# olegroshka/vae-channel-dynamics

Measured on AMD Instinct MI355X. Metric: images/sec SDXL-VAE train step @256x256 (tracking on), higher is better.
Workload: dtype f32

## Files before the change

vae-channel-dynamics_amd/csrc/wgrad3_upwino.hip:

```cpp
#include "wino_common.h"
#include <algorithm>
#include <type_traits>

#ifndef VAE_UPWGRAD_X3
#define VAE_UPWGRAD_X3 1
#endif
#if VAE_UPWGRAD_X3
#include "bf16_frag.h"
#endif
#ifndef VAE_UPWGRAD_PRIO
#define VAE_UPWGRAD_PRIO 1
#endif

namespace {

constexpr int GCI = 32, GCO = 128, NPOS = 9, GNT = 512, GNB = GCO / 32;
constexpr int XSX = 12;
constexpr int XSY = 20;
constexpr int SXF = 3 * GCI * XSX;
constexpr int SYF = 2 * GCO * XSY;
constexpr int GSTAGE = SXF + SYF;
#if VAE_UPWGRAD_X3
constexpr int GPAIR = 2 * GSTAGE;
constexpr int GLDS = 2 * GPAIR * (int)sizeof(float);
extern __shared__ __attribute__((aligned(16))) float upwgrad_lds[];
#endif

__global__ __launch_bounds__(GNT, 2) void wgrad3_upwino_kernel(vae_wgrad_args p, int strips, int64_t nunits) {
#if VAE_UPWGRAD_X3
  float* const smem = upwgrad_lds;
#else
  __shared__ __attribute__((aligned(16))) float smem[2 * GSTAGE];
#endif

  const int tid = threadIdx.x, lane = tid & 63, wave = tid >> 6;
  const int lr = lane & 31, lh = lane >> 5;
  const vae_conv_geom g = p.g;
  const int tilesN = p.N / GCI, ntile = tilesN * (p.M / GCO);
  const wino::SplitTile wg = wino::split_tile_of_workgroup<false>(blockIdx.x, p.nsplit, ntile);
  const int tile = wg.tile, split = wg.split;
  const int tm = tile / tilesN, tn = tile % tilesN;
  const int m0 = tm * GCO, n0 = tn * GCI;
  const wino::UnitRange ur = wino::unit_range(nunits, p.nsplit, split);
  const int64_t ubeg = ur.ubeg;
  const int nu = ur.nu;
  const int upi = g.Hs * strips;
  const bool do_bias = (p.bias_partial != nullptr) && tn == 0;

  const int xx = tid & 15, yq = tid >> 4;
  const bool xrole = tid < 240;
  const int xq = tid & 7, xc = (tid >> 3) % 10, xr = tid / 80;
  const auto rsX = VAE_BUF_RSRC(p.X, (size_t)g.B * g.Hs * g.Ws * g.Cs * 4u);
  const auto rsY = VAE_BUF_RSRC(p.dY, (size_t)g.B * g.Ho * g.Wo * p.ldy * 4u);
  struct Stg {
    f32x4 rx, ry[2];
  };
  const f32x4 z4 = {0.f, 0.f, 0.f, 0.f};
  Stg s0{z4, {z4, z4}}, s1{z4, {z4, z4}};
  f32x4 bsum = z4;
  int ub = (int)(ubeg / upi), urow = (int)((ubeg - (int64_t)ub * upi) / strips), ustrip = (int)((ubeg - (int64_t)ub * upi) % strips);
  const unsigned rowY = (unsigned)g.Wo * p.ldy * 4u;
  auto load_unit = [&](int k, Stg& r) {
    const bool ok = k < nu;
    const int b = ub, i = urow, x0 = ustrip * 8;
    if (++ustrip == strips) {
      ustrip = 0;
      if (++urow == g.Hs) {
        urow = 0;
        ++ub;
      }
    }
    const int hy = i - 1 + xr, hx = x0 - 1 + xc;
    const bool xin = ok && xrole && ((unsigned)hy < (unsigned)g.Hs) && ((unsigned)hx < (unsigned)g.Ws);
    r.rx = VAE_BUF_LOAD4(rsX, xin ? (unsigned)(((b * g.Hs + hy) * g.Ws + hx) * g.Cs + n0 + 4 * xq) * 4u : BUF_OOB);
    const unsigned baseY = (unsigned)((b * g.Ho + 2 * i) * g.Wo + 2 * x0 + xx) * (unsigned)p.ldy * 4u + (unsigned)(m0 + 4 * yq) * 4u;
#pragma unroll
    for (int a = 0; a < 2; ++a) r.ry[a] = VAE_BUF_LOAD4(rsY, ok ? baseY + a * rowY : BUF_OOB);
  };
  auto store_unit = [&](float* st, const Stg& r) {
    float* sx = st;
    float* sy = st + SXF;
    if (xrole) {
#pragma unroll
      for (int e = 0; e < 4; ++e) sx[(xr * GCI + 4 * xq + e) * XSX + xc] = r.rx[e];
    }
#pragma unroll
    for (int a = 0; a < 2; ++a) {
#pragma unroll
      for (int e = 0; e < 4; ++e) sy[(a * GCO + 4 * yq + e) * XSY + xx] = r.ry[a][e];
      if (do_bias) bsum += r.ry[a];
    }
  };

  f32x16 acc[GNB], accx;
#pragma unroll
  for (int nb = 0; nb < GNB; ++nb)
#pragma unroll
    for (int e = 0; e < 16; ++e) acc[nb][e] = 0.f;
#pragma unroll
  for (int e = 0; e < 16; ++e) accx[e] = 0.f;

#if VAE_UPWGRAD_X3
  auto stage_pair = [&](float* st, int kp) __attribute__((always_inline)) {
    store_unit(st, s0);
    store_unit(st + GSTAGE, s1);
    load_unit(2 * kp + 2, s0);
    load_unit(2 * kp + 3, s1);
  };
  load_unit(0, s0);
  load_unit(1, s1);
  stage_pair(smem, 0);
  __syncthreads();
#else
  load_unit(0, s0);
  store_unit(smem, s0);
  load_unit(1, s1);
  __syncthreads();
#endif

  auto build_a = [&](auto PR, auto PC, const float* cx, f32x4& a4) {
    constexpr int pr = decltype(PR)::value, pc = decltype(PC)::value;
    constexpr int vr1 = pr == 0 ? 0 : 1, vr2 = pr == 0 ? 1 : 2;
    const int voff1 = (vr1 * GCI + lr) * XSX + 4 * lh, voff2 = (vr2 * GCI + lr) * XSX + 4 * lh;
    float rc[8];
#pragma unroll
    for (int c = 0; c < 2; ++c) {
      const f32x4 u1 = *reinterpret_cast<const f32x4*>(&cx[voff1 + 4 * c]);
      if (pr == 1) {
#pragma unroll
        for (int e = 0; e < 4; ++e) rc[4 * c + e] = u1[e];
      } else {
        const f32x4 u2 = *reinterpret_cast<const f32x4*>(&cx[voff2 + 4 * c]);
#pragma unroll
        for (int e = 0; e < 4; ++e) rc[4 * c + e] = u1[e] - u2[e];
      }
    }
#pragma unroll
    for (int e = 0; e < 4; ++e) a4[e] = pc == 0 ? rc[e] - rc[e + 1] : (pc == 1 ? rc[e + 1] : rc[e + 1] - rc[e + 2]);
  };
  auto build_b = [&](auto PR, auto PC, const float* cy, int nb, f32x4& b4) {
    constexpr int pr = decltype(PR)::value, pc = decltype(PC)::value;
    constexpr int dr1 = pr == 2 ? 1 : 0;
    const int doff = (dr1 * GCO + nb * 32 + lr) * XSY + 8 * lh;
    float rc[8];
#pragma unroll
    for (int c = 0; c < 2; ++c) {
      const f32x4 d0 = *reinterpret_cast<const f32x4*>(&cy[doff + 4 * c]);
      if (pr == 1) {
        const f32x4 d1 = *reinterpret_cast<const f32x4*>(&cy[doff + GCO * XSY + 4 * c]);
#pragma unroll
        for (int e = 0; e < 4; ++e) rc[4 * c + e] = d0[e] + d1[e];
      } else {
#pragma unroll
        for (int e = 0; e < 4; ++e) rc[4 * c + e] = d0[e];
      }
    }
#pragma unroll
    for (int e = 0; e < 4; ++e) b4[e] = pc == 0 ? rc[2 * e] : (pc == 1 ? rc[2 * e] + rc[2 * e + 1] : rc[2 * e + 1]);
  };
  using I2 = std::integral_constant<int, 2>;

  auto run = [&](auto PR, auto PC, auto EXTRA) {
    constexpr bool extra = decltype(EXTRA)::value;
#if VAE_UPWGRAD_X3
    auto step = [&](int kp) {
      const float* cst = smem + (kp & 1) * GPAIR;
      float* nst = smem + ((kp + 1) & 1) * GPAIR;
      Bf3 a3, bb;
      {
        f32x4 a0, a1;
        build_a(PR, PC, cst, a0);
        build_a(PR, PC, cst + GSTAGE, a1);
        a3 = split8(a0, a1);
      }
      if (extra) stage_pair(nst, kp + 1);
      __builtin_amdgcn_sched_barrier(0);
#pragma unroll
      for (int nb = 0; nb < GNB; ++nb) {
        if (nb == GNB - 1 && !extra) {
          __builtin_amdgcn_sched_barrier(0);
          stage_pair(nst, kp + 1);
          __builtin_amdgcn_sched_barrier(0);
        }
        f32x4 b0, b1;
        build_b(PR, PC, cst + SXF, nb, b0);
        build_b(PR, PC, cst + GSTAGE + SXF, nb, b1);
        bb = split8(b0, b1);
#pragma unroll
        for (int t = 0; t < 6; ++t) acc[nb] = mma_x3_term(t, a3.p, bb.p, acc[nb]);
      }
      if (extra) {
        f32x4 a0, a1, b0, b1;
        build_a(I2{}, I2{}, cst, a0);
        build_a(I2{}, I2{}, cst + GSTAGE, a1);
        build_b(I2{}, I2{}, cst + SXF, wave, b0);
        build_b(I2{}, I2{}, cst + GSTAGE + SXF, wave, b1);
        a3 = split8(a0, a1);
        bb = split8(b0, b1);
#pragma unroll
        for (int t = 0; t < 6; ++t) accx = mma_x3_term(t, a3.p, bb.p, accx);
      }
      __syncthreads();
    };
    const int np = (nu + 1) / 2;
    for (int kp = 0; kp < np; ++kp) step(kp);
#else
    auto step = [&](int k, const Stg& cur, Stg& nxt) {
      const float* cx = smem + (k & 1) * GSTAGE;
      const float* cy = cx + SXF;
      float* nst = smem + ((k + 1) & 1) * GSTAGE;
      f32x4 a4, bb[2];
      build_a(PR, PC, cx, a4);
      build_b(PR, PC, cy, 0, bb[0]);
#pragma unroll
      for (int nb = 0; nb < GNB; ++nb) {
        __builtin_amdgcn_sched_barrier(0);
        if (nb == 1) {
          load_unit(k + 2, nxt);
          __builtin_amdgcn_sched_barrier(0);
        }
        if (nb + 1 < GNB) build_b(PR, PC, cy, nb + 1, bb[(nb + 1) & 1]);
#pragma unroll
        for (int e = 0; e < 4; ++e) acc[nb] = __builtin_amdgcn_mfma_f32_32x32x2f32(a4[e], bb[nb & 1][e], acc[nb], 0, 0, 0);
        __builtin_amdgcn_sched_barrier(0);
      }
      if (extra) {
        f32x4 ax, bx;
        build_a(I2{}, I2{}, cx, ax);
        build_b(I2{}, I2{}, cy, wave, bx);
#pragma unroll
        for (int e = 0; e < 4; ++e) accx = __builtin_amdgcn_mfma_f32_32x32x2f32(ax[e], bx[e], accx, 0, 0, 0);
      }
      store_unit(nst, cur);
      __syncthreads();
    };
    int k = 0;
    for (; k + 1 < nu; k += 2) {
      step(k, s1, s0);
      step(k + 1, s0, s1);
    }
    if (k < nu) step(k, s1, s0);
#endif
  };
#if VAE_UPWGRAD_X3 && VAE_UPWGRAD_PRIO
  if (__builtin_amdgcn_readfirstlane(tid) >= 256) __builtin_amdgcn_s_setprio(1);
#endif
  {
    using I0 = std::integral_constant<int, 0>;
    using I1 = std::integral_constant<int, 1>;
    using T = std::true_type;
    using F_ = std::false_type;
    switch (wave) {
      case 0: run(I0{}, I0{}, T{}); break;
      case 1: run(I0{}, I1{}, T{}); break;
      case 2: run(I0{}, I2{}, T{}); break;
      case 3: run(I1{}, I0{}, T{}); break;
      case 4: run(I1{}, I1{}, F_{}); break;
      case 5: run(I1{}, I2{}, F_{}); break;
      case 6: run(I2{}, I0{}, F_{}); break;
      default: run(I2{}, I1{}, F_{}); break;
    }
  }
#if VAE_UPWGRAD_X3 && VAE_UPWGRAD_PRIO
  __builtin_amdgcn_s_setprio(0);
#endif

  float* __restrict__ O = p.partial + (int64_t)split * NPOS * p.N * p.M;
  wino::slab_store<GNB>(O, wave, p.N, p.M, n0, m0, 0, acc, lr, lh);
  if (wave < 4) wino::slab_store<1>(O, 8, p.N, p.M, n0, m0, wave, &accx, lr, lh);
  if (do_bias) wino::bias_tail(bsum, xx, p.bias_partial, (int64_t)split * p.M + m0 + 4 * yq);
}

}

bool wgrad3_upwino_eligible(const vae_wgrad_args& a) {
  const vae_conv_geom& g = a.g;
  if (!wino::wgrad_eligible_common(a, GCI, GCO) || a.x_bf16 || a.y_bf16 || a.xf != VAE_XF_NONE) return false;
  if (g.mode != VAE_MODE_UP2X || g.Ho != 2 * g.Hs || g.Wo != 2 * g.Ws) return false;
  return g.Ws % 8 == 0 && g.Cs >= a.N;
}

int64_t wgrad3_upwino_units(const vae_conv_geom& g) { return (int64_t)g.B * g.Hs * (g.Ws / 8); }

int launch_wgrad3_upwino(const vae_wgrad_args& a, hipStream_t st) {
  const vae_conv_geom& g = a.g;
  const int64_t nunits = wgrad3_upwino_units(g);
  dim3 grid((unsigned)((a.M / GCO) * (a.N / GCI) * a.nsplit), 1, 1);
#if VAE_UPWGRAD_X3
  VAE_RESERVE_LDS(wgrad3_upwino_kernel, GLDS, "wgrad3_upwino");
  hipLaunchKernelGGL(wgrad3_upwino_kernel, grid, dim3(GNT), GLDS, st, a, g.Ws / 8, nunits);
#else
  hipLaunchKernelGGL(wgrad3_upwino_kernel, grid, dim3(GNT), 0, st, a, g.Ws / 8, nunits);
#endif
  return 0;
}
```

Baseline: 120.0.

## Software-pipeline B-operand builds under MFMA in upsample Winograd wgrad kernel

Adds a pipelined step for the x3 bf16 path of the upsample Winograd weight-gradient kernel. The B operand for the next column block is built from LDS while the current block's MFMAs run, using a double-buffered register operand. Explicit sched_group_barrier patterns interleave MFMA, LDS reads and VALU work, and s_setprio raises wave priority around the MFMA section. This targets LDS-read and split latency sitting between matrix ops, at the cost of more live registers and a compiler-schedule-sensitive instruction mix.

```diff
diff --git a/vae-channel-dynamics_amd/csrc/wgrad3_upwino.hip b/vae-channel-dynamics_amd/csrc/wgrad3_upwino.hip
--- a/vae-channel-dynamics_amd/csrc/wgrad3_upwino.hip
+++ b/vae-channel-dynamics_amd/csrc/wgrad3_upwino.hip
@@ -10,6 +10,12 @@
 #endif
 #ifndef VAE_UPWGRAD_PRIO
 #define VAE_UPWGRAD_PRIO 1
+#endif
+#ifndef VAE_UPWGRAD_PIPE_PRIO
+#define VAE_UPWGRAD_PIPE_PRIO 1
+#endif
+#ifndef VAE_UPWGRAD_PIPE
+#define VAE_UPWGRAD_PIPE 1
 #endif
 
 namespace {
@@ -163,6 +169,71 @@
   auto run = [&](auto PR, auto PC, auto EXTRA) {
     constexpr bool extra = decltype(EXTRA)::value;
 #if VAE_UPWGRAD_X3
+#if VAE_UPWGRAD_PIPE
+    auto step = [&](int kp) {
+      const float* cst = smem + (kp & 1) * GPAIR;
+      float* nst = smem + ((kp + 1) & 1) * GPAIR;
+      Bf3 a3, ax3, bb[2];
+      auto operand = [&](auto PR_, auto PC_, int nb, Bf3& o) {
+        f32x4 b0, b1;
+        build_b(PR_, PC_, cst + SXF, nb, b0);
+        build_b(PR_, PC_, cst + GSTAGE + SXF, nb, b1);
+        o = split8(b0, b1);
+      };
+      {
+        f32x4 a0, a1;
+        build_a(PR, PC, cst, a0);
+        build_a(PR, PC, cst + GSTAGE, a1);
+        a3 = split8(a0, a1);
+      }
+      if (extra) stage_pair(nst, kp + 1);
+      operand(PR, PC, 0, bb[0]);
+      __builtin_amdgcn_sched_barrier(0);
+      if (VAE_UPWGRAD_PIPE_PRIO && extra) __builtin_amdgcn_s_setprio(2);
+      constexpr int pr = decltype(PR)::value, pc = decltype(PC)::value;
+      constexpr int nrd = pr == 1 ? 4 : 2;
+      constexpr int gv = (44 + (pr == 1 ? 16 : 0) + (pc == 1 ? 8 : 0) + 5) / 6;
+#pragma unroll
+      for (int nb = 0; nb < GNB; ++nb) {
+        if (nb == GNB - 1 && !extra) {
+          stage_pair(nst, kp + 1);
+          __builtin_amdgcn_sched_barrier(0);
+        }
+        if (nb + 1 < GNB) {
+          operand(PR, PC, nb + 1, bb[(nb + 1) & 1]);
+        } else if (extra) {
+          f32x4 a0, a1;
+          build_a(I2{}, I2{}, cst, a0);
+          build_a(I2{}, I2{}, cst + GSTAGE, a1);
+          ax3 = split8(a0, a1);
+          operand(I2{}, I2{}, wave, bb[0]);
+        }
+#pragma unroll
+        for (int t = 0; t < 6; ++t) acc[nb] = mma_x3_term(t, a3.p, bb[nb & 1].p, acc[nb]);
+        if (nb + 1 < GNB) {
+#pragma unroll
+          for (int i = 0; i < 6; ++i) {
+            __builtin_amdgcn_sched_group_barrier(0x008, 1, 0);
+            if (i < 2) __builtin_amdgcn_sched_group_barrier(0x100, nrd, 0);
+            __builtin_amdgcn_sched_group_barrier(0x002, gv, 0);
+          }
+        } else if (extra) {
+#pragma unroll
+          for (int i = 0; i < 6; ++i) {
+            __builtin_amdgcn_sched_group_barrier(0x008, 1, 0);
+            if (i < 1) __builtin_amdgcn_sched_group_barrier(0x100, 12, 0);
+            __builtin_amdgcn_sched_group_barrier(0x002, 19, 0);
+          }
+#pragma unroll
+          for (int t = 0; t < 6; ++t) accx = mma_x3_term(t, ax3.p, bb[0].p, accx);
+          __builtin_amdgcn_sched_group_barrier(0x008, 6, 0);
+        }
+        __builtin_amdgcn_sched_barrier(0);
+      }
+      if (VAE_UPWGRAD_PIPE_PRIO && extra) __builtin_amdgcn_s_setprio(0);
+      __syncthreads();
+    };
+#else
     auto step = [&](int kp) {
       const float* cst = smem + (kp & 1) * GPAIR;
       float* nst = smem + ((kp + 1) & 1) * GPAIR;
@@ -202,6 +273,7 @@
       }
       __syncthreads();
     };
+#endif
     const int np = (nu + 1) / 2;
     for (int kp = 0; kp < np; ++kp) step(kp);
 #else
```

Result: no change. 119.1 (-0.7%).
